# tianyili2017/HEVC-Complexity-Reduction

Measured on AMD Instinct MI355X. Metric: CTUs/sec (ETH-CNN inference), higher is better.
Workload: dtype f32; 1 GPU; All-Intra 3840x2160 QP32, 50 frames synthetic YUV; width=3840, height=2160, frames_per_gpu=50, qp=32, ranks=1, devices_visible=1, rank0_device=0, one_rank_per_device=True, device=AMD Radeon Graphics (gfx950:sramecc+:xnack-, 256 CUs), host NUMA node 0

## Files before the change

### hevc-complexity-reduction_amd/csrc/ethcnn_kernels.h

```cpp
#pragma once
#include <hip/hip_runtime.h>

#include "ethcnn_spec.h"

namespace ethcnn {

struct Workspace {
    int cap = 0;
    uint4* xs = nullptr;
    uint4* xm = nullptr;
    uint4* xl = nullptr;
    float* feat = nullptr;
    uint16_t* featb = nullptr;
    float* h1 = nullptr;
    float* h2 = nullptr;
    float* logits = nullptr;
    float* raw = nullptr;
    int* flags = nullptr;
    int flags_cap = 0;
};

struct FrameGeom {
    int width, height;
    long pitch, frame_stride;
    int cw, ch, nctu;
};

void launch_tile(const uint8_t* d_luma, const FrameGeom& g, long ctu0, int n, const Workspace& ws, int n_flags,
                 hipStream_t s, int max_blocks = 0, const unsigned* wait_rows = nullptr, unsigned wait_seq = 0, unsigned* gave_up = nullptr);
void launch_trunk(const Workspace& ws, const DeviceWeights& w, int n, bool resi, hipStream_t s, int fc1_plan = 0);
void launch_trunk_direct(const uint8_t* d_luma, const FrameGeom& g, long ctu0, const Workspace& ws, const DeviceWeights& w, int n, hipStream_t s);
void launch_trunk_f16(const Workspace& ws, const DeviceWeights& w, int n, hipStream_t s, bool ml_only = false);
void launch_trunk_f16_fold(const uint8_t* d_luma, const FrameGeom& g, long ctu0, int n, const Workspace& ws, const DeviceWeights& w, int n_flags,
                           hipStream_t s);
void launch_trunk_f16_foldall(const uint8_t* d_luma, const FrameGeom& g, long ctu0, int n, const Workspace& ws, const DeviceWeights& w, int n_flags,
                              hipStream_t s, int blocks_per_cu = 2);
void launch_fc1(const Workspace& ws, const DeviceWeights& w, int n, float* out, hipStream_t s);
void launch_fc1_fast(const Workspace& ws, const DeviceWeights& w, int n, float* out, int plan, hipStream_t s, int cus = 256);
void launch_heads(const Workspace& ws, const DeviceWeights& w, int n, float qn, int nctu_per_frame,
                  long ctu0, float thr1, float thr2, float* d_probs, hipStream_t s);
void launch_heads_f16(const Workspace& ws, const DeviceWeights& w, int n, float qn, int nctu_per_frame, long ctu0, float thr1, float thr2,
                      float* d_probs, hipStream_t s);
#ifdef ETHCNN_FULL_FENCE
#define ETHCNN_HANDOFF_RELEASE() asm volatile("buffer_wbl2 sc1\n\ts_waitcnt vmcnt(0) lgkmcnt(0)" ::: "memory")
#define ETHCNN_HANDOFF_ACQUIRE() asm volatile("buffer_inv sc1" ::: "memory")
#else
#define ETHCNN_HANDOFF_RELEASE() asm volatile("s_waitcnt vmcnt(0)" ::: "memory")
#define ETHCNN_HANDOFF_ACQUIRE() \
    do {                         \
    } while (0)
#endif

inline int sync_words(int nchunks) { return 2 * nchunks + 8; }
constexpr int kSmallPassMaxCtus = 2304;
bool small_pass_ok(const uint8_t* d_luma, const FrameGeom& g, int n);
int small_pass_sync_words(int n, int nchunks);
void launch_small_pass(const uint8_t* d_luma, const FrameGeom& g, long ctu0, int n, bool resi, const Workspace& ws,
                       const DeviceWeights& w, float* fc1_out, float qn, float thr1, float thr2, float* d_probs, int nchunks,
                       int* d_sync, int epoch, unsigned* done, unsigned done_seq, hipStream_t s, bool pull = false,
                       const unsigned* wait_rows = nullptr, unsigned wait_seq = 0, unsigned* gave_up = nullptr, float* host_probs = nullptr);
void launch_gate(const Workspace& ws, int n, int nctu_per_frame, long ctu0, float thr2, float* d_probs,
                 hipStream_t s);

unsigned lstm_heads_blocks(int n);
int lstm_gate_words(int n);
void launch_lstm(const float* d_vec, const float* d_state_in, float* d_state_out, const float* d_lstm_blob, int n, int qp,
                 int i_frame, float thr1, float thr2, float* d_raw, float* d_probs, int* d_gate, unsigned* done, unsigned done_seq,
                 int one_launch, int epoch, hipStream_t s);
int lstm_frame_words(int n);
constexpr int kLstmOneLaunchMaxCtus = 640;

void launch_mfma_rate(int blocks, int iters, float* d_sink, hipStream_t s);

int chunks_per_frame(int nctu);

struct GateIndex {
    int nctu, cpf, r0, c0;
    float inv_nctu;
};
__device__ __forceinline__ int gate_chunk(const GateIndex& gi, int ctu) {
    const int u = gi.r0 + ctu;
    int f = (int)((float)u * gi.inv_nctu);
    if (f * gi.nctu > u) --f;
    if ((f + 1) * gi.nctu <= u) ++f;
    return f * gi.cpf + (u - f * gi.nctu) / kSubBatch - gi.c0;
}

inline GateIndex make_gate_index(int nctu, long ctu0) {
    GateIndex gi;
    gi.nctu = nctu;
    gi.cpf = chunks_per_frame(nctu);
    gi.r0 = (int)(ctu0 % nctu);
    gi.c0 = gi.r0 / kSubBatch;
    gi.inv_nctu = 1.0f / (float)nctu;
    return gi;
}


}
```

### hevc-complexity-reduction_amd/csrc/ethcnn_pass.cpp

```cpp
#include "ethcnn_ctx.h"

int make_geom(ethcnn_ctx* c, int w, int h, ptrdiff_t pitch, ptrdiff_t fstride, FrameGeom* g) {
    if (w <= 0 || h <= 0) return set_err(c, ETHCNN_ERR_ARG, "bad frame size %dx%d", w, h);
    if (pitch < w) return set_err(c, ETHCNN_ERR_ARG, "pitch %td < width %d", pitch, w);
    g->width = w;
    g->height = h;
    g->pitch = (long)pitch;
    g->frame_stride = (long)fstride;
    g->cw = (w + 63) / 64;
    g->ch = (h + 63) / 64;
    g->nctu = g->cw * g->ch;
    return 0;
}

unsigned done_arm(ethcnn_ctx* c) {
    if (!c->done_sync || !c->h_done) return 0;
    if (++c->done_seq == 0) ++c->done_seq;
    return c->done_seq;
}
hipError_t stream_sync(ethcnn_ctx* c) {
    const unsigned seq = c->done_armed;
    c->done_armed = 0;
    if (seq) {
        const auto t0 = std::chrono::steady_clock::now();
        for (unsigned spins = 1;; ++spins) {
            if (__atomic_load_n(c->h_done, __ATOMIC_ACQUIRE) == seq) return hipSuccess;
#if defined(__SSE2__)
            _mm_pause();
#endif
            if ((spins & 4095u) == 0 && std::chrono::steady_clock::now() - t0 > std::chrono::milliseconds(5)) break;
        }
    }
    return hipStreamSynchronize(c->stream);
}

int serial_end(ethcnn_ctx* c) {
    c->main_dirty = true;
    return 0;
}

int run_small_pass(ethcnn_ctx* c, const uint8_t* d_luma, const FrameGeom& g, long ctu0, int n, bool resi, const Workspace& w,
                   float* fc1_out, float qn, float* d_probs, int nchunks, bool pull, const unsigned* wait_rows) {
    const int words = small_pass_sync_words(n, nchunks);
    c->done_armed = 0;
    if (c->small_epoch >= (1 << 30)) c->ssync_clean = false;
    if (words > c->ssync_cap || !c->ssync_clean) {
        if (words > c->ssync_cap) {
            HIPCHK(c, hipStreamSynchronize(c->stream));
            if (c->d_ssync) (void)hipFree(c->d_ssync);
            c->d_ssync = nullptr;
            c->ssync_cap = 0;
            const int cap = words;
            HIPCHK(c, hipMalloc((void**)&c->d_ssync, (size_t)cap * sizeof(int)));
            c->ssync_cap = cap;
        }
        HIPCHK(c, hipMemsetAsync(c->d_ssync, 0, (size_t)c->ssync_cap * sizeof(int), c->stream));
        c->small_epoch = 0;
    }
    ++c->small_epoch;
    c->ssync_clean = false;
    (void)hipGetLastError();
    const unsigned seq = resi ? 0u : done_arm(c);
    { StageTimer t(c, ETHCNN_STAGE_FC1, n); launch_small_pass(d_luma, g, ctu0, n, resi, w, c->dw, fc1_out, qn, c->thr1, c->thr2, d_probs, nchunks, c->d_ssync, c->small_epoch, seq ? c->h_done : nullptr, seq, c->stream, pull, wait_rows, c->rows_seq, c->h_done + 1, (seq && !resi) ? c->host_probs : nullptr); }
    const hipError_t le = hipGetLastError();
    if (le != hipSuccess) return set_err(c, ETHCNN_ERR_DEVICE, "launch of the single-launch small pass failed: %s", hipGetErrorString(le));
    c->ssync_clean = true;
    c->done_armed = seq;
    c->host_probs_used = seq && !resi && c->host_probs != nullptr && reinterpret_cast<uintptr_t>(c->host_probs) % 16 == 0;
    return 0;
}

int run_pass(ethcnn_ctx* c, const uint8_t* d_luma, const FrameGeom& g, long ctu0, int n, int qp, float* d_probs_pass,
             hipEvent_t input_ready) {
    const int cpf = chunks_per_frame(g.nctu);
    const long nchunks = (ctu0 + n - 1) / g.nctu * cpf + ((ctu0 + n - 1) % g.nctu) / kSubBatch + 1 -
                         (ctu0 / g.nctu * cpf + (ctu0 % g.nctu) / kSubBatch);
    c->done_armed = 0;
    const bool takes_small = c->small_launch && n < kPipelineMinCtus && small_pass_ok(d_luma, g, n);
    int rc = (c->fc1_plan && !takes_small) ? ensure_fast_weights(c, c->fc1_plan) : 0;
    if (rc) return rc;
    rc = ensure_workspace(c, n, (int)nchunks);
    if (rc) return rc;
    const float qn = (float)qp * (1.0f / 51.0f);
    static const int fold3_knob = [] { const char* e = dev_env("ETHCNN_PLAN3_FOLD"); return e ? std::atoi(e) : 2; }();
    const bool fold3 = c->fc1_plan == 3 && fold3_knob != 0 && c->tile_wait_rows == nullptr;
    const bool side_tile = c->overlap != 0 && n >= kPipelineMinCtus && !fold3;
    const int p = side_tile ? (int)(c->pass_idx++ & 1) : 0;
    const Workspace w = ws_view(c, p);
    if (side_tile && !c->s_tile && (rc = ensure_side_streams(c)) != 0) return rc;
    hipStream_t s_tile = side_tile ? c->s_tile : c->stream;
    if (input_ready) HIPCHK(c, hipStreamWaitEvent(s_tile, input_ready, 0));
    if (!side_tile && c->small_launch && small_pass_ok(d_luma, g, n)) {
        Workspace wv = w;
        if (!c->debug_capture) wv.h2 = wv.logits = wv.raw = nullptr;
        rc = run_small_pass(c, d_luma, g, ctu0, n, false, wv, w.h1, qn, d_probs_pass, (int)nchunks, c->luma_over_pcie,
                            c->luma_over_pcie ? c->tile_wait_rows : nullptr);
        if (rc) return rc;
        c->main_dirty = true;
        c->times.ctus += n;
        c->last_n = n;
        c->last_parity = p;
        c->last_fast = 0;
        return 0;
    }
    if (side_tile) {
        HIPCHK(c, hipStreamWaitEvent(s_tile, c->e_trunk[p], 0));
        if (c->main_dirty) {
            HIPCHK(c, hipEventRecord(c->e_main, c->stream));
            c->main_dirty = false;
        }
        HIPCHK(c, hipStreamWaitEvent(s_tile, c->e_main, 0));
        const bool behind_fc1 = c->tile_after_fc1 != 0 && c->fc1_plan != 0;
        HIPCHK(c, hipStreamWaitEvent(s_tile, behind_fc1 ? c->e_fc1[p ^ 1] : c->e_trunk[p ^ 1], 0));
    }
    static const bool fold_knob = [] { const char* e = dev_env("ETHCNN_TILE_FOLD"); return e && std::atoi(e) != 0; }();
    const bool fold = fold_knob && c->fc1_plan == 0 && (g.width % 16 == 0) && (g.pitch % 16 == 0) && (g.frame_stride % 16 == 0) &&
                      (reinterpret_cast<uintptr_t>(d_luma) % 16 == 0);
    (void)hipGetLastError();
#define LAUNCH_OK(name)                                                                                            \
    do {                                                                                                           \
        const hipError_t le_ = hipGetLastError();                                                                  \
        if (le_ != hipSuccess) return set_err(c, ETHCNN_ERR_DEVICE, "launch of the %s stage failed: %s", name, hipGetErrorString(le_)); \
    } while (0)
    static const int only_knob = [] { const char* e = dev_env("ETHCNN_STAGE_ONLY"); return e ? std::atoi(e) : 0; }();
    static int passes_seen = 0;
    const int only = (only_knob != 0 && ++passes_seen > 3) ? only_knob : 0;
    if (fold3 || (only != 0 && only != 1)) {
    } else if (fold) {
        HIPCHK(c, hipMemsetAsync(w.flags, 0, (size_t)sync_words((int)nchunks) * sizeof(int), s_tile));
    } else {
        StageTimer t(c, ETHCNN_STAGE_TILE, n, s_tile);
        launch_tile(d_luma, g, ctu0, n, w, sync_words((int)nchunks), s_tile, side_tile ? c->tile_blocks : 0,
                    side_tile ? nullptr : c->tile_wait_rows, c->rows_seq, c->h_done + 1);
    }
    LAUNCH_OK("tile");
    if (side_tile) {
        HIPCHK(c, hipEventRecord(c->e_tile[p], s_tile));
        HIPCHK(c, hipStreamWaitEvent(c->stream, c->e_tile[p], 0));
    }
    const int fast = c->fc1_plan;
    if (only == 0 || only == 1)
    { StageTimer t(c, ETHCNN_STAGE_TRUNK);
      if (fold) launch_trunk_direct(d_luma, g, ctu0, w, c->dw, n, c->stream);
      else if (fold3 && fold3_knob == 1) {
          launch_trunk_f16_fold(d_luma, g, ctu0, n, w, c->dw, sync_words((int)nchunks), c->stream);
          launch_trunk_f16(w, c->dw, n, c->stream, true);
      } else if (fold3) {
          static const int bpc = [] { const char* e = dev_env("ETHCNN_PLAN3_FOLD_BLOCKS"); return e ? std::atoi(e) : 2; }();
          launch_trunk_f16_foldall(d_luma, g, ctu0, n, w, c->dw, sync_words((int)nchunks), c->stream, bpc);
      } else if (fast == 3) launch_trunk_f16(w, c->dw, n, c->stream);
      else launch_trunk(w, c->dw, n, false, c->stream, fast); }
    LAUNCH_OK("trunk");
    if (side_tile) HIPCHK(c, hipEventRecord(c->e_trunk[p], c->stream));
    Workspace wv = w;
    if (!c->debug_capture) wv.h2 = wv.logits = wv.raw = nullptr;
    if (fast) {
        if (only == 0 || only == 2) { StageTimer t(c, ETHCNN_STAGE_FC1, n); launch_fc1_fast(w, c->dw, n, w.h1, fast == 3 ? 2 : fast, c->stream, c->cus); }
        LAUNCH_OK("FC1 (16-bit pipe)");
        if (side_tile && c->tile_after_fc1) HIPCHK(c, hipEventRecord(c->e_fc1[p], c->stream));
        static const bool heads16_knob = [] { const char* e = dev_env("ETHCNN_PLAN3_HEADS"); return !e || std::atoi(e) != 0; }();
        if (only == 0 || only == 3) { StageTimer t(c, ETHCNN_STAGE_HEADS);
          if (fast == 3 && heads16_knob && c->dw.heads16_w)
              launch_heads_f16(wv, c->dw, n, qn, g.nctu, ctu0, c->thr1, c->thr2, d_probs_pass, c->stream);
          else launch_heads(wv, c->dw, n, qn, g.nctu, ctu0, c->thr1, c->thr2, d_probs_pass, c->stream); }
    } else {
        if (only == 0 || only == 2) { StageTimer t(c, ETHCNN_STAGE_FC1, n); launch_fc1(w, c->dw, n, w.h1, c->stream); }
        LAUNCH_OK("FC1");
        if (only == 0 || only == 3) { StageTimer t(c, ETHCNN_STAGE_HEADS); launch_heads(wv, c->dw, n, qn, g.nctu, ctu0, c->thr1, c->thr2, d_probs_pass, c->stream); }
    }
    if (only == 0 || only == 3) { StageTimer t(c, ETHCNN_STAGE_GATE); launch_gate(w, n, g.nctu, ctu0, c->thr2, d_probs_pass, c->stream); }
    LAUNCH_OK("heads / gate");
#undef LAUNCH_OK
    if (!side_tile) c->main_dirty = true;
    c->times.ctus += n;
    c->last_n = n;
    c->last_parity = p;
    c->last_fast = fast;
    return 0;
}

std::vector<Pass> plan_passes(int nctu, int nframes, int max_ctus) {
    std::vector<Pass> out;
    if (nctu <= max_ctus) {
        const int fpp = std::max(1, max_ctus / nctu);
        for (int f = 0; f < nframes; f += fpp) {
            const int nf = std::min(fpp, nframes - f);
            out.push_back({(long)f * nctu, nf * nctu});
        }
    } else {
        for (int f = 0; f < nframes; ++f)
            for (int o = 0; o < nctu; o += max_ctus) out.push_back({(long)f * nctu + o, std::min(max_ctus, nctu - o)});
    }
    return out;
}

static void calibration_picture(std::vector<uint8_t>& luma, int w, int h) {
    luma.resize((size_t)w * h);
    uint64_t s = 0x9E3779B97F4A7C15ull;
    auto rnd = [&]() { s ^= s << 13; s ^= s >> 7; s ^= s << 17; return (uint32_t)(s >> 32); };
    for (int ty = 0; ty < h / 128; ++ty)
        for (int tx = 0; tx < w / 128; ++tx) {
            const int kind = (tx + 5 * ty) % 6, base = 16 + (int)(rnd() % 208), amp = 1 + (int)(rnd() % 6), per = 4 << (rnd() % 4);
            for (int y = 0; y < 128; ++y)
                for (int x = 0; x < 128; ++x) {
                    int v;
                    switch (kind) {
                        case 0: v = base; break;
                        case 1: v = base + (int)(rnd() % (2 * amp + 1)) - amp; break;
                        case 2: v = (x * 2 + y) % 256; break;
                        case 3: v = (int)(rnd() & 255); break;
                        case 4: v = ((x / per) & 1) ? 235 : 20; break;
                        default: { const int a = x % (2 * per), b = y % (2 * per);
                                   v = 128 + (a < per ? a : 2 * per - a) * 96 / per - 48 + (b < per ? b : 2 * per - b) * 32 / per - 16; }
                    }
                    luma[(size_t)(ty * 128 + y) * w + tx * 128 + x] = (uint8_t)std::min(255, std::max(0, v));
                }
        }
}
int calibrate_fast_plan(ethcnn_ctx* c, int plan, double* max_abs) {
    constexpr int W = 2048, H = 1280;
    constexpr int kQps[2] = {22, 37};
    FrameGeom g;
    int rc = make_geom(c, W, H, W, (ptrdiff_t)W * H, &g);
    if (rc) return rc;
    std::vector<uint8_t> luma;
    calibration_picture(luma, W, H);
    const size_t pf = (size_t)g.nctu * kNOut;
    uint8_t* d_luma = nullptr;
    float* d_p = nullptr;
    HIPCHK(c, hipMalloc((void**)&d_luma, luma.size()));
    if (hipMalloc((void**)&d_p, 4 * pf * 4) != hipSuccess) { (void)hipFree(d_luma); return set_err(c, ETHCNN_ERR_NOMEM, "calibration: out of device memory"); }
    std::vector<float> p(4 * pf);
    const float t1 = c->thr1, t2 = c->thr2;
    const int plan0 = c->fc1_plan, small0 = c->small_launch;
    const bool cap0 = c->debug_capture, pcie0 = c->luma_over_pcie;
    const unsigned* const wait0 = c->tile_wait_rows;
    float* const hp0 = c->host_probs;
    c->thr1 = c->thr2 = -1.0f;
    c->small_launch = 0;
    c->debug_capture = false;
    c->tile_wait_rows = nullptr;
    c->luma_over_pcie = false;
    c->host_probs = nullptr;
    hipError_t e = hipMemcpyAsync(d_luma, luma.data(), luma.size(), hipMemcpyHostToDevice, c->stream);
    for (int k = 0; k < 4 && rc == 0 && e == hipSuccess; ++k) {
        c->fc1_plan = (k & 1) == 0 ? 0 : plan;
        rc = run_pass(c, d_luma, g, 0, g.nctu, kQps[k >> 1], d_p + k * pf);
    }
    c->thr1 = t1; c->thr2 = t2; c->fc1_plan = plan0; c->small_launch = small0; c->debug_capture = cap0;
    c->tile_wait_rows = wait0; c->luma_over_pcie = pcie0; c->host_probs = hp0;
    if (rc == 0 && e == hipSuccess) e = hipMemcpyAsync(p.data(), d_p, 4 * pf * 4, hipMemcpyDeviceToHost, c->stream);
    const hipError_t e2 = hipStreamSynchronize(c->stream);
    (void)hipFree(d_luma);
    (void)hipFree(d_p);
    if (rc) return rc;
    if (e != hipSuccess || e2 != hipSuccess) return set_err(c, ETHCNN_ERR_DEVICE, "calibration of plan %d failed: %s", plan, hipGetErrorString(e != hipSuccess ? e : e2));
    double worst = 0.0;
    for (int q = 0; q < 2; ++q)
        for (size_t i = 0; i < pf; ++i) {
            const double d = std::fabs((double)p[(2 * q) * pf + i] - (double)p[(2 * q + 1) * pf + i]);
            if (!(d <= worst)) worst = d;
        }
    *max_abs = worst;
    return ETHCNN_OK;
}

extern "C" int ethcnn_predict_luma_device(ethcnn_ctx* c, const uint8_t* d_luma, int w, int h, ptrdiff_t pitch,
                                          ptrdiff_t fstride, int nframes, int qp, float* d_probs) {
    if (!c || !d_luma || !d_probs || nframes < 0) return c ? set_err(c, ETHCNN_ERR_ARG, "null pointer / negative frame count") : ETHCNN_ERR_ARG;
    if (!c->have_weights) return set_err(c, ETHCNN_ERR_NOWEIGHTS, "no weights loaded");
    FrameGeom g;
    int rc = make_geom(c, w, h, pitch, fstride, &g);
    if (rc) return rc;
    if (nframes == 0) return ETHCNN_OK;
    HIPCHK(c, hipSetDevice(c->device));
    for (const Pass& p : plan_passes(g.nctu, nframes, c->max_ctus)) {
        rc = run_pass(c, d_luma, g, p.ctu0, p.n, qp, d_probs + (size_t)p.ctu0 * kNOut);
        if (rc) return rc;
    }
    return ETHCNN_OK;
}
```

### hevc-complexity-reduction_amd/csrc/ethcnn_trunk.hip

```cpp
#include <hip/hip_runtime.h>

#include <cstdlib>

#include "ethcnn_kernels.h"
#include "ethcnn_trunk_task.h"

namespace ethcnn {

template <bool RESI, int FAST = 0>
__global__ __launch_bounds__(256) void k1_trunk(const uint4* __restrict__ XS, const uint4* __restrict__ XM,
                                                const uint4* __restrict__ XL, int N, int bS, int bM,
                                                const float* __restrict__ wfrag, const float* __restrict__ bfrag,
                                                float* __restrict__ F, float fscale) {
    __shared__ float wl[RESI ? kTrunkResiLds : kTrunkWFrags * 64];
    const int w = __builtin_amdgcn_readfirstlane(threadIdx.x >> 6);
    const int b = blockIdx.x;
    const int groups = (N + 15) / 16;
    if (b < bS) Trunk<0, RESI, false, false, FAST>::run(XS, groups * 16, b * 4 + w, bS * 4, wfrag, bfrag, F, N, wl, nullptr, nullptr, 0, nullptr, fscale);
    else if (b < bS + bM) Trunk<1, RESI, false, false, FAST>::run(XM, groups * 4, (b - bS) * 4 + w, bM * 4, wfrag, bfrag, F, N, wl, nullptr, nullptr, 0, nullptr, fscale);
    else Trunk<2, RESI, false, false, FAST>::run(XL, groups, (b - bS - bM) * 4 + w, (int)(gridDim.x - bS - bM) * 4, wfrag, bfrag, F, N, wl, nullptr, nullptr, 0, nullptr, fscale);
}

#ifndef TRUNK_SH_S
#define TRUNK_SH_S 193
#define TRUNK_SH_M 50
#define TRUNK_SH_L 13
#endif

__global__ __launch_bounds__(256) void k1_trunk_direct(DirectSrc src, int N, int bS, int bM, const float* __restrict__ wfrag,
                                                       const float* __restrict__ bfrag, float* __restrict__ F) {
    __shared__ float wl[kTrunkWFrags * 64 + 8 * 64 * 4];
    const int w = __builtin_amdgcn_readfirstlane(threadIdx.x >> 6);
    const int b = blockIdx.x;
    const int groups = (N + 15) / 16;
    if (b < bS) Trunk<0, false, true>::run(nullptr, groups * 16, b * 4 + w, bS * 4, wfrag, bfrag, F, N, wl, &src);
    else if (b < bS + bM) Trunk<1, false, true>::run(nullptr, groups * 4, (b - bS) * 4 + w, bM * 4, wfrag, bfrag, F, N, wl, &src);
    else Trunk<2, false, true>::run(nullptr, groups, b - bS - bM, 1 << 30, wfrag, bfrag, F, N, wl, &src);
}

void launch_trunk_direct(const uint8_t* d_luma, const FrameGeom& g, long ctu0, const Workspace& ws, const DeviceWeights& w, int n, hipStream_t s) {
    const int groups = (n + 15) / 16, tS = groups * 16, tM = groups * 4;
    auto blocks = [](int tasks, int budget) { int b = (tasks + 3) / 4; return b < budget ? b : budget; };
    const int bS = blocks(tS, TRUNK_SH_S * 3), bM = blocks(tM, TRUNK_SH_M * 3);
    DirectSrc src;
    src.luma = d_luma; src.width = g.width; src.height = g.height; src.pitch = g.pitch; src.frame_stride = g.frame_stride;
    src.cw = g.cw; src.nctu = g.nctu; src.ctu0 = ctu0; src.n_total = n;
    hipLaunchKernelGGL(k1_trunk_direct, dim3(bS + bM + groups), dim3(256), 0, s, src, n, bS, bM, w.trunk_w, w.trunk_b, ws.feat);
}

void launch_trunk(const Workspace& ws, const DeviceWeights& w, int n, bool resi, hipStream_t s, int fc1_plan) {
    const int groups = (n + 15) / 16, tS = groups * 16, tM = groups * 4, tL = groups;
    auto blocks = [](int tasks, int budget) { int b = (tasks + 3) / 4; return b < budget ? b : budget; };
    static int per_cu = 0;
    if (!per_cu) { const char* e = dev_env("ETHCNN_TRUNK_BLOCKS_PER_CU"); per_cu = e ? atoi(e) : 3; }
    const int bS = blocks(tS, TRUNK_SH_S * per_cu), bM = blocks(tM, TRUNK_SH_M * per_cu), bL = blocks(tL, TRUNK_SH_L * per_cu);
    if (fc1_plan == 2)
        hipLaunchKernelGGL((k1_trunk<false, 2>), dim3(bS + bM + bL), dim3(256), 0, s, ws.xs, ws.xm, ws.xl, n, bS, bM,
                           w.trunk_w, w.trunk_b, reinterpret_cast<float*>(ws.featb), w.fast_scale_a);
    else if (resi)
        hipLaunchKernelGGL(k1_trunk<true>, dim3(bS + bM + bL), dim3(256), 0, s, ws.xs, ws.xm, ws.xl, n, bS, bM,
                           w.trunk_w, w.trunk_b, ws.feat, 1.0f);
    else
        hipLaunchKernelGGL(k1_trunk<false>, dim3(bS + bM + bL), dim3(256), 0, s, ws.xs, ws.xm, ws.xl, n, bS, bM,
                           w.trunk_w, w.trunk_b, ws.feat, 1.0f);
}

}
```

### hevc-complexity-reduction_amd/csrc/ethcnn_trunk_task.h

```cpp
#pragma once
#include <hip/hip_runtime.h>

#include "ethcnn_fc1_tile.h"
#include "ethcnn_heads_pass.h"
#include "ethcnn_kernels.h"

namespace ethcnn {

#ifndef TRUNK_BUF_LOADS
#define TRUNK_BUF_LOADS 1
#endif
#ifndef TRUNK_BUF_STORES
#define TRUNK_BUF_STORES 1
#endif

__device__ __forceinline__ f32x4 lrelu4(f32x4 h) {
    const float t0 = 0.2f * h[0], t1 = 0.2f * h[1], t2 = 0.2f * h[2], t3 = 0.2f * h[3];
    float o0, o1, o2, o3;
    asm volatile("v_max_f32 %0, %4, %8\n\tv_max_f32 %1, %5, %9\n\tv_max_f32 %2, %6, %10\n\tv_max_f32 %3, %7, %11\n\ts_nop 1"
                 : "=&v"(o0), "=&v"(o1), "=&v"(o2), "=&v"(o3)
                 : "v"(t0), "v"(t1), "v"(t2), "v"(t3), "v"(h[0]), "v"(h[1]), "v"(h[2]), "v"(h[3]));
    return (f32x4){o0, o1, o2, o3};
}

template <bool RESI>
__device__ __forceinline__ float px_value(int s, int cnt) {
    if (RESI) return ((float)(s - 128 * cnt) / 255.0f) * 10.0f;
    return (float)s * (1.0f / 255.0f);
}

struct DirectSrc {
    const uint8_t* luma;
    int width, height;
    long pitch, frame_stride;
    int cw, nctu;
    long ctu0;
    int n_total;
};

typedef float f32x2 __attribute__((ext_vector_type(2)));
typedef _Float16 f16x2 __attribute__((ext_vector_type(2)));
template <bool SC1>
__device__ __forceinline__ void store_pair_f16x2(const f32x4& qa, const f32x4& qb, float scale, __amdgpu_buffer_rsrc_t rF, int voff) {
    float r[8] = {qa[0] * scale, qa[1] * scale, qa[2] * scale, qa[3] * scale, qb[0] * scale, qb[1] * scale, qb[2] * scale, qb[3] * scale};
#pragma unroll
    for (int p = 0; p < 2; ++p) {
        u32x4 P;
#pragma unroll
        for (int i = 0; i < 4; ++i) {
            const f16x2 h = __builtin_convertvector((f32x2){r[2 * i], r[2 * i + 1]}, f16x2);
            P[i] = __builtin_bit_cast(unsigned, h);
            if (p == 0) {
                r[2 * i] -= (float)h[0];
                r[2 * i + 1] -= (float)h[1];
            }
        }
        __builtin_amdgcn_raw_buffer_store_b128(P, rF, voff + p * 1024, 0, SC1 ? kAuxSc1 : 0);
    }
}

template <int BR, bool RESI, bool DIRECT = false, bool SC1 = false, int FAST = 0>
struct Trunk {
    static constexpr int FCH = 2 * 1024;
    static constexpr int POOL = (BR == 0) ? 1 : (BR == 1 ? 2 : 4);
    static constexpr float SCALE = 1.0f / (float)(POOL * POOL);
    static constexpr float C255S = (1.0f / 255.0f) * SCALE;
    static constexpr int NB = (BR == 0) ? 4 : (BR == 1 ? 2 : 1);
    static constexpr int OFF2 = (BR == 0) ? 672 : (BR == 1 ? 2208 : 2592);
    static constexpr int OFF3 = (BR == 0) ? 0 : (BR == 1 ? 512 : 640);
    static constexpr int NJ = (BR == 0) ? 4 : 8;
    static constexpr int TAB = 255 * POOL * POOL + 1;

    static __device__ __forceinline__ int raw_sum(const uint4 (&raw)[NJ]) {
        int T = 0;
#pragma unroll
        for (int j = 0; j < NJ; ++j) {
            const uint32_t w[4] = {raw[j].x, raw[j].y, raw[j].z, raw[j].w};
#pragma unroll
            for (int i = 0; i < 4; ++i) {
                if (BR == 0) T = (int)__builtin_amdgcn_udot4(w[i], 0x01010101u, (unsigned)T, false);
                else T += (int)((w[i] & 0xffffu) + (w[i] >> 16));
            }
        }
        return T;
    }
    static __device__ __forceinline__ void decode_q2(const uint4 (&raw)[NJ], int q2, float (&x)[4][4], const float* tab) {
        if (BR == 0) {
            const uint32_t w[4] = {raw[q2].x, raw[q2].y, raw[q2].z, raw[q2].w};
#pragma unroll
            for (int q1 = 0; q1 < 4; ++q1)
#pragma unroll
                for (int kx = 0; kx < 4; ++kx) {
                    const int s = (int)((w[q1] >> (8 * kx)) & 0xff);
                    x[q1][kx] = RESI ? tab[s] : (float)s;
                }
        } else {
#pragma unroll
            for (int jj = 0; jj < 2; ++jj) {
                const uint4 rw = raw[2 * q2 + jj];
                const uint32_t w[4] = {rw.x, rw.y, rw.z, rw.w};
#pragma unroll
                for (int hh = 0; hh < 2; ++hh)
#pragma unroll
                    for (int kx = 0; kx < 4; ++kx) {
                        const int s = (int)((w[2 * hh + (kx >> 1)] >> (16 * (kx & 1))) & 0xffff);
                        x[2 * jj + hh][kx] = RESI ? tab[s] : (float)s;
                    }
            }
        }
    }

    struct LaneCtu {
        const uint8_t* base;
        int y0, x0, by, bx;
    };
    static __device__ __forceinline__ LaneCtu lane_ctu(const DirectSrc& S, int task, int lane) {
        const int c = lane & 15;
        int grp;
        LaneCtu L;
        if (BR == 0) { grp = task >> 4; L.by = (task >> 2) & 3; L.bx = task & 3; }
        else if (BR == 1) { grp = task >> 2; L.by = (task >> 1) & 1; L.bx = task & 1; }
        else { grp = task; L.by = 0; L.bx = 0; }
        const int n = grp * 16 + c;
        L.base = nullptr;
        L.y0 = L.x0 = 0;
        if (n < S.n_total) {
            const long gn = S.ctu0 + n;
            const long f = gn / S.nctu;
            const int rr = (int)(gn - f * S.nctu);
            const int cy = rr / S.cw, cx = rr - cy * S.cw;
            L.y0 = cy * 64;
            L.x0 = cx * 64;
            L.base = S.luma + f * S.frame_stride + (long)L.y0 * S.pitch + L.x0;
        }
        return L;
    }
    static __device__ __forceinline__ uint4 direct_record(const DirectSrc& S, const LaneCtu& L, int g, int j) {
        auto in = [&](int Y, int X) { return L.base != nullptr && L.y0 + Y < S.height && L.x0 + X < S.width; };
        auto ld8 = [&](int Y, int X) -> uint2 {
            return in(Y, X) ? *reinterpret_cast<const uint2*>(L.base + (long)Y * S.pitch + X) : make_uint2(0u, 0u);
        };
        auto ld16 = [&](int Y, int X) -> uint4 {
            return in(Y, X) ? *reinterpret_cast<const uint4*>(L.base + (long)Y * S.pitch + X) : make_uint4(0u, 0u, 0u, 0u);
        };
        if (BR == 0) {
            const int Y = 16 * L.by + 8 * (j >> 1) + g, X = 16 * L.bx + 8 * (j & 1);
            const uint2 a = ld8(Y, X), b = ld8(Y + 4, X);
            return make_uint4(a.x, a.y, b.x, b.y);
        }
        uint32_t out[4];
        if (BR == 1) {
            const int q2 = j >> 1, pr = 8 * (q2 >> 1) + 4 * (j & 1) + g, pc = 8 * (q2 & 1);
            const uint4 a = ld16(32 * L.by + 2 * pr, 32 * L.bx + 2 * pc), b = ld16(32 * L.by + 2 * pr + 1, 32 * L.bx + 2 * pc);
            const uint32_t aw[4] = {a.x, a.y, a.z, a.w}, bw[4] = {b.x, b.y, b.z, b.w};
#pragma unroll
            for (int hh = 0; hh < 2; ++hh) {
                const uint32_t a0 = aw[2 * hh], a1 = aw[2 * hh + 1], b0 = bw[2 * hh], b1 = bw[2 * hh + 1];
                const uint32_t s0 = __builtin_amdgcn_udot4(a0, 0x00000101u, __builtin_amdgcn_udot4(b0, 0x00000101u, 0u, false), false);
                const uint32_t s1 = __builtin_amdgcn_udot4(a0, 0x01010000u, __builtin_amdgcn_udot4(b0, 0x01010000u, 0u, false), false);
                const uint32_t s2 = __builtin_amdgcn_udot4(a1, 0x00000101u, __builtin_amdgcn_udot4(b1, 0x00000101u, 0u, false), false);
                const uint32_t s3 = __builtin_amdgcn_udot4(a1, 0x01010000u, __builtin_amdgcn_udot4(b1, 0x01010000u, 0u, false), false);
                out[2 * hh] = s0 | (s1 << 16);
                out[2 * hh + 1] = s2 | (s3 << 16);
            }
            return make_uint4(out[0], out[1], out[2], out[3]);
        }
#pragma unroll
        for (int hh = 0; hh < 2; ++hh) {
            const int dd = 2 * j + hh, q2 = dd >> 2, q1 = dd & 3;
            const int pr = 8 * (q2 >> 1) + 4 * (q1 >> 1) + g, pc = 8 * (q2 & 1) + 4 * (q1 & 1);
            uint32_t sacc[4] = {0u, 0u, 0u, 0u};
#pragma unroll
            for (int ry = 0; ry < 4; ++ry) {
                const uint4 v = ld16(4 * pr + ry, 4 * pc);
                sacc[0] = __builtin_amdgcn_udot4(v.x, 0x01010101u, sacc[0], false);
                sacc[1] = __builtin_amdgcn_udot4(v.y, 0x01010101u, sacc[1], false);
                sacc[2] = __builtin_amdgcn_udot4(v.z, 0x01010101u, sacc[2], false);
                sacc[3] = __builtin_amdgcn_udot4(v.w, 0x01010101u, sacc[3], false);
            }
            out[2 * hh] = sacc[0] | (sacc[1] << 16);
            out[2 * hh + 1] = sacc[2] | (sacc[3] << 16);
        }
        return make_uint4(out[0], out[1], out[2], out[3]);
    }
    static __device__ __forceinline__ bool load_direct(const DirectSrc& S, int task, int lane, uint4 (&raw)[NJ], uint4* xl) {
        const LaneCtu L = lane_ctu(S, task, lane);
        const int g = lane >> 4;
        if (BR != 2) {
#pragma unroll
            for (int j = 0; j < NJ; ++j) raw[j] = direct_record(S, L, g, j);
            return true;
        }
        const int q = __builtin_amdgcn_readfirstlane((int)(threadIdx.x >> 6));
        xl[(2 * q) * 64 + lane] = direct_record(S, L, g, 2 * q);
        xl[(2 * q + 1) * 64 + lane] = direct_record(S, L, g, 2 * q + 1);
        __syncthreads();
        if (q != 0) return false;
#pragma unroll
        for (int j = 0; j < NJ; ++j) raw[j] = xl[j * 64 + lane];
        return true;
    }

    struct NoWait { __device__ __forceinline__ bool operator()() const { return false; } };
    template <class Ready = NoWait>
    static __device__ __forceinline__ void run(const uint4* __restrict__ X, int ntasks, int wave, int nwaves,
                                               const float* __restrict__ wfrag, const float* __restrict__ bfrag,
                                               float* __restrict__ F, int N, float* wl, const DirectSrc* src = nullptr,
                                               int* claim = nullptr, int tag = 0, int* s_owned = nullptr, float fscale = 1.0f,
                                               Ready ready = Ready()) {
        int lane = threadIdx.x & 63;
        if (SC1) asm volatile("" : "+v"(lane));
        const int col = lane & 15, g = lane >> 4;
        if (claim != nullptr && threadIdx.x == 0)
            *s_owned = (__hip_atomic_exchange(claim, tag, __ATOMIC_RELAXED, __HIP_MEMORY_SCOPE_AGENT) != tag);
        uint4 raw[NJ];
        bool active = wave < ntasks;
        if (DIRECT && active) active = load_direct(*src, wave, lane, raw, reinterpret_cast<uint4*>(wl + kTrunkWFrags * 64));
        f32x4 B1, B2[2], B3[2];
        {
            const float* bf = bfrag + (size_t)BR * kTrunkBFrags * 64 + lane;
#pragma unroll
            for (int r = 0; r < 4; ++r) B1[r] = bf[r * 64];
#pragma unroll
            for (int t = 0; t < 2; ++t)
#pragma unroll
                for (int r = 0; r < 4; ++r) {
                    B2[t][r] = bf[(4 + t * 4 + r) * 64];
                    B3[t][r] = bf[(12 + t * 4 + r) * 64];
                }
        }
        auto stage = [&]() {
            const float* wf = wfrag + (size_t)BR * kTrunkWFrags * 64;
            for (int i = threadIdx.x; i < kTrunkWFrags * 64; i += 256) wl[i] = wf[i];
            if (RESI)
                for (int i = threadIdx.x; i < TAB; i += 256) wl[kTrunkResiTabAt + i] = px_value<true>(i, POOL * POOL) * (BR == 0 ? 1.0f : SCALE);
            __syncthreads();
        };
        stage();
        if (ready()) stage();
        if (claim != nullptr && !*s_owned) return;
        if (!active) return;
        const float* tab = wl + kTrunkResiTabAt;
        const float* wA2 = wl + 4 * 64 + lane;
        const float* wA3 = wl + 36 * 64 + lane;

        float A1[4];
#pragma unroll
        for (int s = 0; s < 4; ++s) A1[s] = wl[s * 64 + lane];

        const int lane16 = lane * 16;
        const int lane_off = FAST ? (g >> 1) * FCH + (g & 1) * 512 + col * 16
                                  : (col * 4 + g * 64) * 4;
        const __amdgpu_buffer_rsrc_t rX = __builtin_amdgcn_make_buffer_rsrc(const_cast<uint4*>(X), 0, -1, 0x00020000);
        const __amdgpu_buffer_rsrc_t rF = __builtin_amdgcn_make_buffer_rsrc(F, 0, -1, 0x00020000);
        if (!DIRECT) {
#pragma unroll
            for (int j = 0; j < NJ; ++j)
                raw[j] = (TRUNK_BUF_LOADS || SC1) ? __builtin_bit_cast(uint4, __builtin_amdgcn_raw_buffer_load_b128(rX, lane16, (wave * NJ + j) * 1024, SC1 ? kAuxSc1 : 0))
                                         : X[((size_t)wave * NJ + j) * 64 + lane];
        }

        for (int task = wave; task < ntasks; task += nwaves) {
            int T = raw_sum(raw);
            T += __shfl_xor(T, 16);
            T += __shfl_xor(T, 32);
            const float mean = px_value<RESI>(T, 256 * POOL * POOL) * (SCALE * (1.0f / 256.0f));
            const float negmean = -mean;

            int grp, by, bx;
            if (BR == 0) { grp = task >> 4; by = (task >> 2) & 3; bx = task & 3; }
            else if (BR == 1) { grp = task >> 2; by = (task >> 1) & 1; bx = task & 1; }
            else { grp = task; by = 0; bx = 0; }
            const bool valid = grp * 16 + col < N;
            const int Fg = grp * (kNFeat * 16 * 4);
            const int Tpos = (BR == 0) ? (task & 15) : (BR == 1 ? 16 + (task & 3) : 20);
            const int Fb = (grp >> 1) * (kFastChunks * FCH) + Tpos * 8 * FCH + (grp & 1) * 256;
            auto store_pair = [&](const f32x4& qa, const f32x4& qb, int pair) {
                store_pair_f16x2<SC1>(qa, qb, fscale, rF, lane_off + Fb + pair * 2 * FCH);
            };

#define CONV1(q2, c1)                                                                                  \
    {                                                                                                  \
        _Pragma("unroll") for (int q1 = 0; q1 < 4; ++q1) c1[q1] = B1;                                  \
        _Pragma("unroll") for (int s = 0; s < 4; ++s)                                                  \
            _Pragma("unroll") for (int q1 = 0; q1 < 4; ++q1) {                                         \
                const float xv = x[q1][s];                                                  \
                c1[q1] = MFMA16(A1[s], RESI ? xv - mean : fmaf(xv, C255S, negmean), c1[q1]);           \
            }                                                                                          \
    }
#define CONV2(c1, c2)                                                                                  \
    {                                                                                                  \
        c2[0] = B2[0];                                                                                 \
        c2[1] = B2[1];                                                                                 \
        _Pragma("unroll") for (int q1 = 0; q1 < 4; ++q1)                                               \
            _Pragma("unroll") for (int r = 0; r < 4; ++r) {                                            \
                c2[0] = MFMA16(wA2[(4 * q1 + r) * 64], c1[q1][r], c2[0]);                                   \
                c2[1] = MFMA16(wA2[(16 + 4 * q1 + r) * 64], c1[q1][r], c2[1]);                                   \
            }                                                                                          \
    }
#define LEAKY1(c1) { _Pragma("unroll") for (int q1 = 0; q1 < 4; ++q1) c1[q1] = lrelu4(c1[q1]); }
#define FINISH2(q2, c2)                                                                                \
    {                                                                                                  \
        a2[q2][0] = lrelu4(c2[0]);                                                                     \
        a2[q2][1] = lrelu4(c2[1]);                                                                     \
        if (FAST) {                                                                                    \
            if (((q2) & 1) && valid) store_pair(a2[(q2) - 1][0], a2[q2][0], (q2) >> 1);                \
        } else if (valid) {                                                                            \
            const int slot = (2 * by + ((q2) >> 1)) * (2 * NB) + 2 * bx + ((q2) & 1);                  \
            const int dst = Fg + ((OFF2 + slot * 24) >> 2) * 256;                                      \
            if (TRUNK_BUF_STORES) {                                                                    \
                __builtin_amdgcn_raw_buffer_store_b128(__builtin_bit_cast(u32x4, a2[q2][0]), rF, lane_off + dst, 0, SC1 ? kAuxSc1 : 0);  \
                if (g < 2) __builtin_amdgcn_raw_buffer_store_b128(__builtin_bit_cast(u32x4, a2[q2][1]), rF, lane_off + dst + 1024, 0, SC1 ? kAuxSc1 : 0); \
            } else {                                                                                   \
                char* p_ = reinterpret_cast<char*>(F) + (size_t)dst + lane_off;                        \
                *reinterpret_cast<f32x4*>(p_) = a2[q2][0];                                             \
                if (g < 2) *reinterpret_cast<f32x4*>(p_ + 1024) = a2[q2][1];                           \
            }                                                                                          \
        }                                                                                              \
    }
            f32x4 a2[4][2];
            f32x4 c3[2] = {B3[0], B3[1]};
#pragma unroll
            for (int q2 = 0; q2 < 4; ++q2) {
                f32x4 c1[4], c2[2];
                float x[4][4];
                decode_q2(raw, q2, x, tab);
                CONV1(q2, c1);
                LEAKY1(c1);
                CONV2(c1, c2);
                FINISH2(q2, c2);
            }
            if (task + nwaves < ntasks) {
                if (DIRECT) {
                    if (BR != 2) (void)load_direct(*src, task + nwaves, lane, raw, nullptr);
                } else {
#pragma unroll
                    for (int j = 0; j < NJ; ++j)
                        raw[j] = (TRUNK_BUF_LOADS || SC1) ? __builtin_bit_cast(uint4, __builtin_amdgcn_raw_buffer_load_b128(rX, lane16, ((task + nwaves) * NJ + j) * 1024, SC1 ? kAuxSc1 : 0))
                                                 : X[((size_t)(task + nwaves) * NJ + j) * 64 + lane];
                }
            }
#undef CONV1
#undef CONV2
#undef LEAKY1
#undef FINISH2
#pragma unroll
            for (int q2 = 0; q2 < 4; ++q2)
#pragma unroll
                for (int r = 0; r < 4; ++r) {
                    c3[0] = MFMA16(wA3[(4 * q2 + r) * 64], a2[q2][0][r], c3[0]);
                    c3[1] = MFMA16(wA3[(24 + 4 * q2 + r) * 64], a2[q2][0][r], c3[1]);
                }
            f32x4 zq[2];
#pragma unroll
            for (int j = 0; j < 2; ++j)
#pragma unroll
                for (int r = 0; r < 4; ++r) {
                    const float hi = __shfl(a2[2 * j + 1][1][r], lane & 31);
                    const float z = (lane < 32) ? a2[2 * j][1][r] : hi;
                    if (FAST) zq[j][r] = z;
                    c3[0] = MFMA16(wA3[(16 + 4 * j + r) * 64], z, c3[0]);
                    c3[1] = MFMA16(wA3[(24 + 16 + 4 * j + r) * 64], z, c3[1]);
                }
            if (FAST) {
                if (valid) {
                    store_pair(zq[0], zq[1], 2);
                    store_pair(lrelu4(c3[0]), lrelu4(c3[1]), 3);
                }
            } else if (valid) {
                const int dst = Fg + ((OFF3 + (by * NB + bx) * 32) >> 2) * 256;
                if (TRUNK_BUF_STORES) {
                    __builtin_amdgcn_raw_buffer_store_b128(__builtin_bit_cast(u32x4, lrelu4(c3[0])), rF, lane_off + dst, 0, SC1 ? kAuxSc1 : 0);
                    __builtin_amdgcn_raw_buffer_store_b128(__builtin_bit_cast(u32x4, lrelu4(c3[1])), rF, lane_off + dst + 1024, 0, SC1 ? kAuxSc1 : 0);
                } else {
                    char* p_ = reinterpret_cast<char*>(F) + (size_t)dst + lane_off;
                    *reinterpret_cast<f32x4*>(p_) = lrelu4(c3[0]);
                    *reinterpret_cast<f32x4*>(p_ + 1024) = lrelu4(c3[1]);
                }
            }
        }
    }
};


}
```

Before: 41.57 million CTU/s.

## Fold tile preprocessing into trunk kernel with per-branch wave specialization

Adds a fused trunk kernel that loads luma slabs into LDS, derives the small/medium/large branch inputs on chip, and runs the three trunk branches in specialized waves within a 384-thread block. The separate tile kernel and flags memset are skipped and gate flags are zeroed inside the kernel. The path becomes the default for large passes with fc1_plan 0. The Trunk template is refactored into a reusable per-task routine with a callback for prefetching. It removes a launch and a global round trip of tile data, at the cost of more block-level barriers, higher LDS use, and dropping the side-stream overlap between tiling and trunk.

```diff
diff --git a/hevc-complexity-reduction_amd/csrc/ethcnn_kernels.h b/hevc-complexity-reduction_amd/csrc/ethcnn_kernels.h
--- a/hevc-complexity-reduction_amd/csrc/ethcnn_kernels.h
+++ b/hevc-complexity-reduction_amd/csrc/ethcnn_kernels.h
@@ -29,7 +29,8 @@
 void launch_tile(const uint8_t* d_luma, const FrameGeom& g, long ctu0, int n, const Workspace& ws, int n_flags,
                  hipStream_t s, int max_blocks = 0, const unsigned* wait_rows = nullptr, unsigned wait_seq = 0, unsigned* gave_up = nullptr);
 void launch_trunk(const Workspace& ws, const DeviceWeights& w, int n, bool resi, hipStream_t s, int fc1_plan = 0);
-void launch_trunk_direct(const uint8_t* d_luma, const FrameGeom& g, long ctu0, const Workspace& ws, const DeviceWeights& w, int n, hipStream_t s);
+void launch_trunk_fold(const uint8_t* d_luma, const FrameGeom& g, long ctu0, int n, const Workspace& ws, const DeviceWeights& w, int n_flags,
+                       hipStream_t s);
 void launch_trunk_f16(const Workspace& ws, const DeviceWeights& w, int n, hipStream_t s, bool ml_only = false);
 void launch_trunk_f16_fold(const uint8_t* d_luma, const FrameGeom& g, long ctu0, int n, const Workspace& ws, const DeviceWeights& w, int n_flags,
                            hipStream_t s);
diff --git a/hevc-complexity-reduction_amd/csrc/ethcnn_pass.cpp b/hevc-complexity-reduction_amd/csrc/ethcnn_pass.cpp
--- a/hevc-complexity-reduction_amd/csrc/ethcnn_pass.cpp
+++ b/hevc-complexity-reduction_amd/csrc/ethcnn_pass.cpp
@@ -84,7 +84,9 @@
     const float qn = (float)qp * (1.0f / 51.0f);
     static const int fold3_knob = [] { const char* e = dev_env("ETHCNN_PLAN3_FOLD"); return e ? std::atoi(e) : 2; }();
     const bool fold3 = c->fc1_plan == 3 && fold3_knob != 0 && c->tile_wait_rows == nullptr;
-    const bool side_tile = c->overlap != 0 && n >= kPipelineMinCtus && !fold3;
+    const bool big = c->overlap != 0 && n >= kPipelineMinCtus;
+    const bool fold = big && c->fc1_plan == 0 && c->tile_wait_rows == nullptr && !c->luma_over_pcie && !c->debug_capture;
+    const bool side_tile = big && !fold3 && !fold;
     const int p = side_tile ? (int)(c->pass_idx++ & 1) : 0;
     const Workspace w = ws_view(c, p);
     if (side_tile && !c->s_tile && (rc = ensure_side_streams(c)) != 0) return rc;
@@ -113,9 +115,6 @@
         const bool behind_fc1 = c->tile_after_fc1 != 0 && c->fc1_plan != 0;
         HIPCHK(c, hipStreamWaitEvent(s_tile, behind_fc1 ? c->e_fc1[p ^ 1] : c->e_trunk[p ^ 1], 0));
     }
-    static const bool fold_knob = [] { const char* e = dev_env("ETHCNN_TILE_FOLD"); return e && std::atoi(e) != 0; }();
-    const bool fold = fold_knob && c->fc1_plan == 0 && (g.width % 16 == 0) && (g.pitch % 16 == 0) && (g.frame_stride % 16 == 0) &&
-                      (reinterpret_cast<uintptr_t>(d_luma) % 16 == 0);
     (void)hipGetLastError();
 #define LAUNCH_OK(name)                                                                                            \
     do {                                                                                                           \
@@ -125,9 +124,7 @@
     static const int only_knob = [] { const char* e = dev_env("ETHCNN_STAGE_ONLY"); return e ? std::atoi(e) : 0; }();
     static int passes_seen = 0;
     const int only = (only_knob != 0 && ++passes_seen > 3) ? only_knob : 0;
-    if (fold3 || (only != 0 && only != 1)) {
-    } else if (fold) {
-        HIPCHK(c, hipMemsetAsync(w.flags, 0, (size_t)sync_words((int)nchunks) * sizeof(int), s_tile));
+    if (fold3 || fold || (only != 0 && only != 1)) {
     } else {
         StageTimer t(c, ETHCNN_STAGE_TILE, n, s_tile);
         launch_tile(d_luma, g, ctu0, n, w, sync_words((int)nchunks), s_tile, side_tile ? c->tile_blocks : 0,
@@ -141,7 +138,7 @@
     const int fast = c->fc1_plan;
     if (only == 0 || only == 1)
     { StageTimer t(c, ETHCNN_STAGE_TRUNK);
-      if (fold) launch_trunk_direct(d_luma, g, ctu0, w, c->dw, n, c->stream);
+      if (fold) launch_trunk_fold(d_luma, g, ctu0, n, w, c->dw, sync_words((int)nchunks), c->stream);
       else if (fold3 && fold3_knob == 1) {
           launch_trunk_f16_fold(d_luma, g, ctu0, n, w, c->dw, sync_words((int)nchunks), c->stream);
           launch_trunk_f16(w, c->dw, n, c->stream, true);
diff --git a/hevc-complexity-reduction_amd/csrc/ethcnn_trunk.hip b/hevc-complexity-reduction_amd/csrc/ethcnn_trunk.hip
--- a/hevc-complexity-reduction_amd/csrc/ethcnn_trunk.hip
+++ b/hevc-complexity-reduction_amd/csrc/ethcnn_trunk.hip
@@ -3,6 +3,7 @@
 #include <cstdlib>
 
 #include "ethcnn_kernels.h"
+#include "ethcnn_tile_group.h"
 #include "ethcnn_trunk_task.h"
 
 namespace ethcnn {
@@ -27,25 +28,120 @@
 #define TRUNK_SH_L 13
 #endif
 
-__global__ __launch_bounds__(256) void k1_trunk_direct(DirectSrc src, int N, int bS, int bM, const float* __restrict__ wfrag,
-                                                       const float* __restrict__ bfrag, float* __restrict__ F) {
-    __shared__ float wl[kTrunkWFrags * 64 + 8 * 64 * 4];
-    const int w = __builtin_amdgcn_readfirstlane(threadIdx.x >> 6);
-    const int b = blockIdx.x;
-    const int groups = (N + 15) / 16;
-    if (b < bS) Trunk<0, false, true>::run(nullptr, groups * 16, b * 4 + w, bS * 4, wfrag, bfrag, F, N, wl, &src);
-    else if (b < bS + bM) Trunk<1, false, true>::run(nullptr, groups * 4, (b - bS) * 4 + w, bM * 4, wfrag, bfrag, F, N, wl, &src);
-    else Trunk<2, false, true>::run(nullptr, groups, b - bS - bM, 1 << 30, wfrag, bfrag, F, N, wl, &src);
+constexpr int kFoldFrags = 80 * 64;
+template <bool FAST>
+__global__ __launch_bounds__(384) __attribute__((amdgpu_waves_per_eu(3, 3))) void k1_trunk_fold(const uint8_t* __restrict__ luma, int width, int height, long pitch, long frame_stride,
+                                                        int cw, int nctu, int f0, int r0, int N, int* __restrict__ gate_flags, int n_flags,
+                                                        uint4* __restrict__ XL, const float* __restrict__ wfrag, const float* __restrict__ bfrag,
+                                                        float* __restrict__ F) {
+    __shared__ float wl[3][kFoldFrags];
+    __shared__ uint32_t tile[16 * kSlabCtuPitch];
+    if (blockIdx.x == 0)
+        for (int i = threadIdx.x; i < n_flags; i += 384) gate_flags[i] = 0;
+    const int t = threadIdx.x, lane = t & 63;
+    const int w = __builtin_amdgcn_readfirstlane(t >> 6);
+    for (int br = 0; br < 3; ++br)
+        for (int i = t; i < kFoldFrags; i += 384) wl[br][i] = wfrag[(br * kTrunkWFrags + 4) * 64 + i];
+    const int ngroups = (N + 15) >> 4;
+    const int col = lane & 15, g = lane >> 4;
+    __syncthreads();
+    if ((int)blockIdx.x >= ngroups) return;
+    if (w < 4) {
+        Trunk<0, false>::Wave W;
+        W.load_bias(bfrag, lane);
+        W.set_operands(wfrag, wl[0], wl[0] + 32 * 64, nullptr, lane);
+        W.set_output(F, N, 1.0f, lane);
+        SlabLoader L;
+        uint4 pre[4];
+        L.init32(t, luma, width, frame_stride, cw, nctu, f0, r0, N, (int)blockIdx.x * 16);
+        L.template load<FAST>(0, pre, width, height, pitch);
+#pragma unroll 1
+        for (int grp = blockIdx.x; grp < ngroups; grp += gridDim.x) {
+#pragma unroll 1
+            for (int s = 0; s < 4; ++s) {
+                L.to_lds(tile, pre);
+                __syncthreads();
+                uint4 raw[4];
+#pragma unroll
+                for (int j = 0; j < 4; ++j) raw[j] = slab_xs_record(tile, col, g, j, w);
+                __syncthreads();
+                Trunk<0, false>::task(W, raw, grp * 16 + 4 * s + w, [&]() {
+                    if (s < 3) {
+                        L.template load<FAST>(s + 1, pre, width, height, pitch);
+                    } else {
+                        const int nx = grp + (int)gridDim.x;
+                        if (nx < ngroups) {
+                            L.init32(t, luma, width, frame_stride, cw, nctu, f0, r0, N, nx * 16);
+                            L.template load<FAST>(0, pre, width, height, pitch);
+                        }
+                    }
+                });
+            }
+        }
+        return;
+    }
+    const int r = w - 4;
+    const __amdgpu_buffer_rsrc_t rL = __builtin_amdgcn_make_buffer_rsrc(XL, 0, -1, 0x00020000);
+    Trunk<1, false>::Wave WM;
+    auto m_consts = [&]() {
+        WM.load_bias(bfrag, lane);
+        WM.set_operands(wfrag + (size_t)kTrunkWFrags * 64, wl[1], wl[1] + 32 * 64, nullptr, lane);
+        WM.set_output(F, N, 1.0f, lane);
+    };
+    m_consts();
+    auto l_task = [&](int grp) {
+        Trunk<2, false>::Wave WL;
+        WL.load_bias(bfrag, lane);
+        WL.set_operands(wfrag + (size_t)2 * kTrunkWFrags * 64, wl[2], wl[2] + 32 * 64, nullptr, lane);
+        WL.set_output(F, N, 1.0f, lane);
+        asm volatile("s_waitcnt vmcnt(0)" ::: "memory");
+        uint4 rawl[8];
+#pragma unroll
+        for (int j = 0; j < 8; ++j)
+            rawl[j] = __builtin_bit_cast(uint4, __builtin_amdgcn_raw_buffer_load_b128(rL, lane * 16, (grp * 8 + j) * 1024, kAuxSc1));
+        Trunk<2, false>::task(WL, rawl, grp, []() {});
+    };
+#pragma unroll 1
+    for (int grp = blockIdx.x; grp < ngroups; grp += gridDim.x) {
+        const bool has_l = (grp & 1) == r;
+#pragma unroll 1
+        for (int uy = 0; uy < 2; ++uy) {
+            uint4 rawm[8];
+#pragma unroll
+            for (int sh = 0; sh < 2; ++sh) {
+                __syncthreads();
+#pragma unroll
+                for (int jj = 0; jj < 4; ++jj) rawm[4 * sh + jj] = slab_xm_record(tile, col, g, 4 * sh + jj, r);
+                if (has_l) {
+#pragma unroll
+                    for (int m = 0; m < 2; ++m) {
+                        const uint4 v = slab_xl_record(tile, col, g, 2 * m + sh);
+                        __builtin_amdgcn_raw_buffer_store_b128((u32x4){v.x, v.y, v.z, v.w}, rL, ((grp * 8 + 4 * uy + 2 * m + sh) * 64 + lane) * 16, 0, kAuxSc1);
+                    }
+                }
+                __syncthreads();
+            }
+            Trunk<1, false>::task(WM, rawm, grp * 4 + 2 * uy + r, []() {});
+        }
+        if (has_l) {
+            l_task(grp);
+            m_consts();
+        }
+    }
 }
 
-void launch_trunk_direct(const uint8_t* d_luma, const FrameGeom& g, long ctu0, const Workspace& ws, const DeviceWeights& w, int n, hipStream_t s) {
-    const int groups = (n + 15) / 16, tS = groups * 16, tM = groups * 4;
-    auto blocks = [](int tasks, int budget) { int b = (tasks + 3) / 4; return b < budget ? b : budget; };
-    const int bS = blocks(tS, TRUNK_SH_S * 3), bM = blocks(tM, TRUNK_SH_M * 3);
-    DirectSrc src;
-    src.luma = d_luma; src.width = g.width; src.height = g.height; src.pitch = g.pitch; src.frame_stride = g.frame_stride;
-    src.cw = g.cw; src.nctu = g.nctu; src.ctu0 = ctu0; src.n_total = n;
-    hipLaunchKernelGGL(k1_trunk_direct, dim3(bS + bM + groups), dim3(256), 0, s, src, n, bS, bM, w.trunk_w, w.trunk_b, ws.feat);
+void launch_trunk_fold(const uint8_t* d_luma, const FrameGeom& g, long ctu0, int n, const Workspace& ws, const DeviceWeights& w, int n_flags,
+                       hipStream_t s) {
+    const int groups = (n + 15) / 16;
+    const int blocks = groups < 512 ? groups : 512;
+    const bool fast = (g.width % 16 == 0) && (g.pitch % 16 == 0) && (g.frame_stride % 16 == 0) && (reinterpret_cast<uintptr_t>(d_luma) % 16 == 0);
+    const int f0 = (int)(ctu0 / g.nctu), r0 = (int)(ctu0 % g.nctu);
+    if (fast)
+        hipLaunchKernelGGL(k1_trunk_fold<true>, dim3(blocks), dim3(384), 0, s, d_luma, g.width, g.height, g.pitch, g.frame_stride, g.cw, g.nctu,
+                           f0, r0, n, ws.flags, n_flags, ws.xl, w.trunk_w, w.trunk_b, ws.feat);
+    else
+        hipLaunchKernelGGL(k1_trunk_fold<false>, dim3(blocks), dim3(384), 0, s, d_luma, g.width, g.height, g.pitch, g.frame_stride, g.cw, g.nctu,
+                           f0, r0, n, ws.flags, n_flags, ws.xl, w.trunk_w, w.trunk_b, ws.feat);
 }
 
 void launch_trunk(const Workspace& ws, const DeviceWeights& w, int n, bool resi, hipStream_t s, int fc1_plan) {
diff --git a/hevc-complexity-reduction_amd/csrc/ethcnn_trunk_task.h b/hevc-complexity-reduction_amd/csrc/ethcnn_trunk_task.h
--- a/hevc-complexity-reduction_amd/csrc/ethcnn_trunk_task.h
+++ b/hevc-complexity-reduction_amd/csrc/ethcnn_trunk_task.h
@@ -201,24 +201,16 @@
         return true;
     }
 
-    struct NoWait { __device__ __forceinline__ bool operator()() const { return false; } };
-    template <class Ready = NoWait>
-    static __device__ __forceinline__ void run(const uint4* __restrict__ X, int ntasks, int wave, int nwaves,
-                                               const float* __restrict__ wfrag, const float* __restrict__ bfrag,
-                                               float* __restrict__ F, int N, float* wl, const DirectSrc* src = nullptr,
-                                               int* claim = nullptr, int tag = 0, int* s_owned = nullptr, float fscale = 1.0f,
-                                               Ready ready = Ready()) {
-        int lane = threadIdx.x & 63;
-        if (SC1) asm volatile("" : "+v"(lane));
-        const int col = lane & 15, g = lane >> 4;
-        if (claim != nullptr && threadIdx.x == 0)
-            *s_owned = (__hip_atomic_exchange(claim, tag, __ATOMIC_RELAXED, __HIP_MEMORY_SCOPE_AGENT) != tag);
-        uint4 raw[NJ];
-        bool active = wave < ntasks;
-        if (DIRECT && active) active = load_direct(*src, wave, lane, raw, reinterpret_cast<uint4*>(wl + kTrunkWFrags * 64));
+    struct Wave {
         f32x4 B1, B2[2], B3[2];
-        {
-            const float* bf = bfrag + (size_t)BR * kTrunkBFrags * 64 + lane;
+        float A1[4];
+        const float *wA2, *wA3, *tab;
+        float* F;
+        __amdgpu_buffer_rsrc_t rF;
+        float fscale;
+        int N, lane, lane_off;
+        __device__ __forceinline__ void load_bias(const float* __restrict__ bfrag, int lane_) {
+            const float* bf = bfrag + (size_t)BR * kTrunkBFrags * 64 + lane_;
 #pragma unroll
             for (int r = 0; r < 4; ++r) B1[r] = bf[r * 64];
 #pragma unroll
@@ -229,38 +221,34 @@
                     B3[t][r] = bf[(12 + t * 4 + r) * 64];
                 }
         }
-        auto stage = [&]() {
-            const float* wf = wfrag + (size_t)BR * kTrunkWFrags * 64;
-            for (int i = threadIdx.x; i < kTrunkWFrags * 64; i += 256) wl[i] = wf[i];
-            if (RESI)
-                for (int i = threadIdx.x; i < TAB; i += 256) wl[kTrunkResiTabAt + i] = px_value<true>(i, POOL * POOL) * (BR == 0 ? 1.0f : SCALE);
-            __syncthreads();
-        };
-        stage();
-        if (ready()) stage();
-        if (claim != nullptr && !*s_owned) return;
-        if (!active) return;
-        const float* tab = wl + kTrunkResiTabAt;
-        const float* wA2 = wl + 4 * 64 + lane;
-        const float* wA3 = wl + 36 * 64 + lane;
-
-        float A1[4];
-#pragma unroll
-        for (int s = 0; s < 4; ++s) A1[s] = wl[s * 64 + lane];
-
-        const int lane16 = lane * 16;
-        const int lane_off = FAST ? (g >> 1) * FCH + (g & 1) * 512 + col * 16
-                                  : (col * 4 + g * 64) * 4;
-        const __amdgpu_buffer_rsrc_t rX = __builtin_amdgcn_make_buffer_rsrc(const_cast<uint4*>(X), 0, -1, 0x00020000);
-        const __amdgpu_buffer_rsrc_t rF = __builtin_amdgcn_make_buffer_rsrc(F, 0, -1, 0x00020000);
-        if (!DIRECT) {
-#pragma unroll
-            for (int j = 0; j < NJ; ++j)
-                raw[j] = (TRUNK_BUF_LOADS || SC1) ? __builtin_bit_cast(uint4, __builtin_amdgcn_raw_buffer_load_b128(rX, lane16, (wave * NJ + j) * 1024, SC1 ? kAuxSc1 : 0))
-                                         : X[((size_t)wave * NJ + j) * 64 + lane];
-        }
-
-        for (int task = wave; task < ntasks; task += nwaves) {
+        __device__ __forceinline__ void set_operands(const float* a1, const float* a2, const float* a3, const float* tab_, int lane_) {
+            tab = tab_;
+            wA2 = a2 + lane_;
+            wA3 = a3 + lane_;
+#pragma unroll
+            for (int s = 0; s < 4; ++s) A1[s] = a1[s * 64 + lane_];
+        }
+        __device__ __forceinline__ void set_output(float* F_, int N_, float fscale_, int lane_) {
+            const int col = lane_ & 15, g = lane_ >> 4;
+            F = F_; N = N_; fscale = fscale_; lane = lane_;
+            lane_off = FAST ? (g >> 1) * FCH + (g & 1) * 512 + col * 16
+                            : (col * 4 + g * 64) * 4;
+            rF = __builtin_amdgcn_make_buffer_rsrc(F_, 0, -1, 0x00020000);
+        }
+    };
+
+    template <class Next>
+    static __device__ __forceinline__ void task(const Wave& W, uint4 (&raw)[NJ], int task, Next next) {
+        const int lane = W.lane, col = lane & 15, g = lane >> 4, lane_off = W.lane_off, N = W.N;
+        const f32x4 B1 = W.B1;
+        const f32x4 B2[2] = {W.B2[0], W.B2[1]}, B3[2] = {W.B3[0], W.B3[1]};
+        const float A1[4] = {W.A1[0], W.A1[1], W.A1[2], W.A1[3]};
+        const float *wA2 = W.wA2, *wA3 = W.wA3, *tab = W.tab;
+        float* const F = W.F;
+        const __amdgpu_buffer_rsrc_t rF = W.rF;
+        const float fscale = W.fscale;
+        (void)F; (void)tab; (void)fscale;
+        {
             int T = raw_sum(raw);
             T += __shfl_xor(T, 16);
             T += __shfl_xor(T, 32);
@@ -330,16 +318,7 @@
                 CONV2(c1, c2);
                 FINISH2(q2, c2);
             }
-            if (task + nwaves < ntasks) {
-                if (DIRECT) {
-                    if (BR != 2) (void)load_direct(*src, task + nwaves, lane, raw, nullptr);
-                } else {
-#pragma unroll
-                    for (int j = 0; j < NJ; ++j)
-                        raw[j] = (TRUNK_BUF_LOADS || SC1) ? __builtin_bit_cast(uint4, __builtin_amdgcn_raw_buffer_load_b128(rX, lane16, ((task + nwaves) * NJ + j) * 1024, SC1 ? kAuxSc1 : 0))
-                                                 : X[((size_t)(task + nwaves) * NJ + j) * 64 + lane];
-                }
-            }
+            next();
 #undef CONV1
 #undef CONV2
 #undef LEAKY1
@@ -380,6 +359,61 @@
             }
         }
     }
+
+    struct NoWait { __device__ __forceinline__ bool operator()() const { return false; } };
+    template <class Ready = NoWait>
+    static __device__ __forceinline__ void run(const uint4* __restrict__ X, int ntasks, int wave, int nwaves,
+                                               const float* __restrict__ wfrag, const float* __restrict__ bfrag,
+                                               float* __restrict__ F, int N, float* wl, const DirectSrc* src = nullptr,
+                                               int* claim = nullptr, int tag = 0, int* s_owned = nullptr, float fscale = 1.0f,
+                                               Ready ready = Ready()) {
+        int lane = threadIdx.x & 63;
+        if (SC1) asm volatile("" : "+v"(lane));
+        if (claim != nullptr && threadIdx.x == 0)
+            *s_owned = (__hip_atomic_exchange(claim, tag, __ATOMIC_RELAXED, __HIP_MEMORY_SCOPE_AGENT) != tag);
+        uint4 raw[NJ];
+        bool active = wave < ntasks;
+        if (DIRECT && active) active = load_direct(*src, wave, lane, raw, reinterpret_cast<uint4*>(wl + kTrunkWFrags * 64));
+        Wave W;
+        W.load_bias(bfrag, lane);
+        auto stage = [&]() {
+            const float* wf = wfrag + (size_t)BR * kTrunkWFrags * 64;
+            for (int i = threadIdx.x; i < kTrunkWFrags * 64; i += 256) wl[i] = wf[i];
+            if (RESI)
+                for (int i = threadIdx.x; i < TAB; i += 256) wl[kTrunkResiTabAt + i] = px_value<true>(i, POOL * POOL) * (BR == 0 ? 1.0f : SCALE);
+            __syncthreads();
+        };
+        stage();
+        if (ready()) stage();
+        if (claim != nullptr && !*s_owned) return;
+        if (!active) return;
+        W.set_operands(wl, wl + 4 * 64, wl + 36 * 64, wl + kTrunkResiTabAt, lane);
+
+        const int lane16 = lane * 16;
+        const __amdgpu_buffer_rsrc_t rX = __builtin_amdgcn_make_buffer_rsrc(const_cast<uint4*>(X), 0, -1, 0x00020000);
+        W.set_output(F, N, fscale, lane);
+        if (!DIRECT) {
+#pragma unroll
+            for (int j = 0; j < NJ; ++j)
+                raw[j] = (TRUNK_BUF_LOADS || SC1) ? __builtin_bit_cast(uint4, __builtin_amdgcn_raw_buffer_load_b128(rX, lane16, (wave * NJ + j) * 1024, SC1 ? kAuxSc1 : 0))
+                                         : X[((size_t)wave * NJ + j) * 64 + lane];
+        }
+
+        for (int task = wave; task < ntasks; task += nwaves) {
+            Trunk::task(W, raw, task, [&]() {
+                if (task + nwaves < ntasks) {
+                    if (DIRECT) {
+                        if (BR != 2) (void)load_direct(*src, task + nwaves, lane, raw, nullptr);
+                    } else {
+#pragma unroll
+                        for (int j = 0; j < NJ; ++j)
+                            raw[j] = (TRUNK_BUF_LOADS || SC1) ? __builtin_bit_cast(uint4, __builtin_amdgcn_raw_buffer_load_b128(rX, lane16, ((task + nwaves) * NJ + j) * 1024, SC1 ? kAuxSc1 : 0))
+                                                     : X[((size_t)(task + nwaves) * NJ + j) * 64 + lane];
+                    }
+                }
+            });
+        }
+    }
 };
 
 
```

Result: slower. 36.25 million CTU/s (-12.8%).
